# szemenyeim/DynEnv

Hardware: AMD Instinct MI355X
Metric: agent-steps/s (higher is better)
Workload: dtype f64

## Files before the change

### dynenv_amd/csrc/driving_kernels.hip

```cpp
#include "driving_dev.h"

__constant__ DrvConst C;

#include "driving_host.h"

struct DrvMailbox {
  double p1x[DRV_NS][2], p1y[DRV_NS][2], p2x[DRV_NS][2], p2y[DRV_NS][2], nx[DRV_NS], ny[DRV_NS];
  int hash[DRV_NS][2], count[DRV_NS], flag[DRV_NS];
};
struct DrvObsStage {
  float carRow[DRV_MAXA][8];
  float goal[DRV_MAXA][2];
  float shared[DRV_MAXO * 4 + DRV_MAXP * 2 + DRV_LANE_ROWS * 5];
};
#ifdef DRV_PROFILE
#define DRV_PROF(...) __VA_ARGS__
#else
#define DRV_PROF(...)
#endif
#define DRV_CLIST 128
struct __align__(16) DrvLds {
  double px[DRV_NB], py[DRV_NB], vx[DRV_NB], vy[DRV_NB], ang[DRV_NB], w[DRV_NB], vbx[DRV_NB], vby[DRV_NB], wb[DRV_NB];
  double minv[DRV_NB], iinv[DRV_NB];
  double rc[16], rs[16], rotAng[16];
  double dirx[16], diry[16], prevx[16], prevy[16], goalx[16], goaly[16];
  double cosRel0[16];
  double dprev[16];
  double cmass[16], cpower[16], chx[16], chy[16];
  double aabb[DRV_MAXA][4];
  int flags[DRV_NB], moving[DRV_NB];
  double ox[DRV_MAXO], oy[DRV_MAXO];
  int s_pair[DRV_NS], s_meta[DRV_NS], s_hash0[DRV_NS], s_hash1[DRV_NS];
  double s_jn0[DRV_NS], s_jt0[DRV_NS], s_jn1[DRV_NS], s_jt1[DRV_NS];
  double rewAcc[16], posAcc[16];
  int lastCand[64];
  int stepErr;
  unsigned char act[16];
  int still[DRV_NB];
  unsigned short clist[DRV_CLIST];
  int clistN;
  int sLvMeta;
  unsigned long long sActive;
  unsigned char sLevel[DRV_NS];
  union {
    DrvMailbox mb;
    DrvObsStage ob;
  } u;
};

static_assert(sizeof(DrvLds) <= 10240, "16 one-wave workgroups per CU - one residency round of 4096 environments on 256 CUs - need <= 160 KB / 16 of LDS each");
__shared__ DrvLds g_L;


#define DRV_COS_PI_2 6.123233995736766e-17
template <int R>
struct RoadK;
template <>
struct RoadK<0> {
  static constexpr double p0x = 875.0, p0y = 0.0, dirx = 0.0, diry = 1.0, lat = 2.0 * 35.0 + 5.0, length = 1000.0;
  static constexpr double dirAngle = 1.5707963267948966, cosDir0 = DRV_COS_PI_2, nx = -1.0, ny = DRV_COS_PI_2;
};
template <>
struct RoadK<1> {
  static constexpr double p0x = 0.0, p0y = 500.0, dirx = 1.0, diry = 0.0, lat = 1.0 * 35.0 + 5.0, length = 1750.0;
  static constexpr double dirAngle = 0.0, cosDir0 = 1.0, nx = DRV_COS_PI_2, ny = 1.0;
};

// ... 73 lines not shown
  const DevSC sc = INL ? dev_sincos_inl(ang) : dev_sincos(ang);
  CarRot r;
  r.c = sc.c; r.s = sc.s;
  r.cosRel0 = INL ? dev_sincos_inl(RoadK<0>::dirAngle - ang).c : dev_cos(RoadK<0>::dirAngle - ang);
  L.rc[lane] = r.c; L.rs[lane] = r.s; L.rotAng[lane] = ang; L.cosRel0[lane] = r.cosRel0;
  static_assert(RoadK<1>::dirAngle == 0.0, "cos(road1.dirAngle - angle) is read from rc");
  return r;
}

struct BoxW {
  V2 v[4], n[4];
};
DE_DEV void box_world(BoxW& b, V2 p, double rc, double rs, double hx, double hy) {
  const double lx[4] = {-hx, hx, hx, -hx}, ly[4] = {-hy, -hy, hy, hy};
  const double nx[4] = {-1.0, 0.0, 1.0, 0.0}, ny[4] = {0.0, -1.0, 0.0, 1.0};
#pragma unroll
  for (int i = 0; i < 4; ++i) {
    b.v[i] = v2(dms_xform_x(rc, rs, lx[i], ly[i], p.x), dms_xform_y(rc, rs, lx[i], ly[i], p.y));
    b.n[i] = v2(rc * nx[i] - rs * ny[i], rs * nx[i] + rc * ny[i]);
  }
}

struct Contacts {
  int count;
  V2 n, p1[2], p2[2];
  int hash[2];
};

struct EdgeW {
  V2 ap, bp, n;
  int ah, bh;
};

struct BoxP {
  V2 p;
  double c, s, hx, hy;
};
DE_DEV V2 boxp_vertex(const BoxP& b, int i) {
  const double lx = (i == 1 || i == 2) ? b.hx : -b.hx;
  const double ly = (i >= 2) ? b.hy : -b.hy;
  return v2(dms_xform_x(b.c, b.s, lx, ly, b.p.x), dms_xform_y(b.c, b.s, lx, ly, b.p.y));
}
DE_DEV V2 boxp_normal(const BoxP& b, int i) {
  const double nx = (i == 0) ? -1.0 : ((i == 2) ? 1.0 : 0.0);
  const double ny = (i == 1) ? -1.0 : ((i == 3) ? 1.0 : 0.0);
  return v2(b.c * nx - b.s * ny, b.s * nx + b.c * ny);
}

template <int S> DE_DEV double quad_bcast(double x) {
  int lo = __double2loint(x), hi = __double2hiint(x);
  lo = __builtin_amdgcn_update_dpp(lo, lo, S * 0x55, 0xF, 0xF, false);
  hi = __builtin_amdgcn_update_dpp(hi, hi, S * 0x55, 0xF, 0xF, false);
  return __hiloint2double(hi, lo);
}
DE_DEV void quad_argmax_first(double v, double& best, int& idx) {
  best = -INFINITY; idx = 0;
  double m;
  m = quad_bcast<0>(v); if (m > best) { best = m; idx = 0; }
  m = quad_bcast<1>(v); if (m > best) { best = m; idx = 1; }
  m = quad_bcast<2>(v); if (m > best) { best = m; idx = 2; }
  m = quad_bcast<3>(v); if (m > best) { best = m; idx = 3; }
}

DE_DEV int poly_support_index(const BoxP& p, V2 n, int q) {
  double mx;
  int index;
  quad_argmax_first(vdot_f(boxp_vertex(p, q), n), mx, index);
  return index;
}

DE_DEV EdgeW support_edge_poly(const BoxP& p, int slot, V2 n, int q) {
  int i1 = poly_support_index(p, n, q);
  int i0 = (i1 + 3) & 3;
  int i2 = (i1 + 1) & 3;
  int h = slot * 4;
  V2 n1 = boxp_normal(p, i1), n2 = boxp_normal(p, i2);
  EdgeW e;
  V2 vm = boxp_vertex(p, i1);
  if (vdot(n, n1) > vdot(n, n2)) {
    e.ap = boxp_vertex(p, i0); e.ah = h + i0; e.bp = vm; e.bh = h + i1; e.n = n1;
  } else {
    e.ap = vm; e.ah = h + i1; e.bp = boxp_vertex(p, i2); e.bh = h + i2; e.n = n2;
  }
  return e;
}

DE_DEV int hash_pair(int a, int b) { return 1 + ((a << 8) | b); }

DE_DEV void contact_points(const EdgeW& e1, const EdgeW& e2, V2 n, Contacts& out) {
  double d_e1_a = vcross(e1.ap, n), d_e1_b = vcross(e1.bp, n);
  double d_e2_a = vcross(e2.ap, n), d_e2_b = vcross(e2.bp, n);
  double e1_denom = 1.0 / (d_e1_b - d_e1_a + DE_DBL_MIN);
  double e2_denom = 1.0 / (d_e2_b - d_e2_a + DE_DBL_MIN);
  out.n = n;
  out.count = 0;
  {
    V2 p1 = vadd(vmul(n, 0.0), vlerp(e1.ap, e1.bp, fclamp01_cp((d_e2_b - d_e1_a) * e1_denom)));
    V2 p2 = vadd(vmul(n, -0.0), vlerp(e2.ap, e2.bp, fclamp01_cp((d_e1_a - d_e2_a) * e2_denom)));
    double dist = vdot(vsub(p2, p1), n);
    if (dist <= 0.0) { out.p1[0] = p1; out.p2[0] = p2; out.hash[0] = hash_pair(e1.ah, e2.bh); out.count = 1; }
  }
  {
    V2 p1 = vadd(vmul(n, 0.0), vlerp(e1.ap, e1.bp, fclamp01_cp((d_e2_a - d_e1_a) * e1_denom)));
    V2 p2 = vadd(vmul(n, -0.0), vlerp(e2.ap, e2.bp, fclamp01_cp((d_e1_b - d_e2_a) * e2_denom)));
    double dist = vdot(vsub(p2, p1), n);
    if (dist <= 0.0) {
      int h = hash_pair(e1.bh, e2.ah);
      if (out.count == 0) { out.p1[0] = p1; out.p2[0] = p2; out.hash[0] = h; }
      else { out.p1[1] = p1; out.p2[1] = p2; out.hash[1] = h; }
      out.count += 1;
    }
  }
}

DE_DEV double sat_max_sep(const BoxP& a, const BoxP& b, int q, int& best) {
  const V2 n = boxp_normal(a, q);
  const double d0 = vdot_f(n, boxp_vertex(a, q));
  double minv = INFINITY;
#pragma unroll
  for (int j = 0; j < 4; ++j) {
    double d = vdot_f(n, boxp_vertex(b, j)) - d0;
    if (d < minv) minv = d;
  }
  double maxsep;
  quad_argmax_first(minv, maxsep, best);
  return maxsep;
}

DE_DEV void poly_to_poly(const BoxP& p1, int slot1, const BoxP& p2, int slot2, int q, Contacts& out) {
  out.count = 0;
  int ia, ib;
  double sa = sat_max_sep(p1, p2, q, ia);
  if (sa > 0.0) return;
  double sb = sat_max_sep(p2, p1, q, ib);
  if (sb > 0.0) return;
  V2 n;
  if (sa >= sb) n = boxp_normal(p1, ia); else n = vneg(boxp_normal(p2, ib));
  const EdgeW e1 = support_edge_poly(p1, slot1, n, q);
  const EdgeW e2 = support_edge_poly(p2, slot2, vneg(n), q);
  contact_points(e1, e2, n, out);
}

DE_DEV void circle_to_poly(V2 c, double r, const BoxP& poly, int q, Contacts& out) {
  out.count = 0;
  double maxsep;
  int best;
  const V2 vq = boxp_vertex(poly, q);
  quad_argmax_first(vdot(boxp_normal(poly, q), vsub(c, vq)), maxsep, best);
  if (maxsep > r) return;
  if (maxsep <= 0.0) {
    V2 fn = boxp_normal(poly, best);
    V2 n = vneg(fn);
    V2 pb = vsub(c, vmul(fn, maxsep));
    out.n = n; out.p1[0] = vadd(c, vmul(n, r)); out.p2[0] = pb; out.hash[0] = 0; out.count = 1;
  } else {
    const V2 a = boxp_vertex(poly, (q + 3) & 3), b = vq;
    const V2 d = vsub(b, a);
    const double t = fclamp01_cp(vdot(d, vsub(c, a)) / vlensq(d));
    const V2 pt = vadd(a, vmul(d, t));
    const double dsq = vlensq(vsub(pt, c));
    double bestd = INFINITY;
    V2 bestp = c;
    double m;
    m = quad_bcast<0>(dsq); if (m < bestd) { bestd = m; bestp = v2(quad_bcast<0>(pt.x), quad_bcast<0>(pt.y)); }
    m = quad_bcast<1>(dsq); if (m < bestd) { bestd = m; bestp = v2(quad_bcast<1>(pt.x), quad_bcast<1>(pt.y)); }
    m = quad_bcast<2>(dsq); if (m < bestd) { bestd = m; bestp = v2(quad_bcast<2>(pt.x), quad_bcast<2>(pt.y)); }
    m = quad_bcast<3>(dsq); if (m < bestd) { bestd = m; bestp = v2(quad_bcast<3>(pt.x), quad_bcast<3>(pt.y)); }
    if (bestd <= r * r) {
      double dist = dm_sqrt(bestd);
      V2 delta = vsub(bestp, c);
      V2 n = (dist != 0.0) ? vmul(delta, 1.0 / dist) : vneg(boxp_normal(poly, best));
      out.n = n; out.p1[0] = vadd(c, vmul(n, r)); out.p2[0] = bestp; out.hash[0] = 0; out.count = 1;
    }
  }
}

struct BodyV {
  V2 p, v, vb;
  double w, wb, minv, iinv;
};
DE_DEV V2 static_pos(const DrvLds& L, int idx) {
  if (idx >= DRV_SLOT_BLD) {
    int k = idx - DRV_SLOT_BLD;
    return v2(DRV_BLD_CX(k), DRV_BLD_CY(k));
  }
  return v2(L.ox[idx - DRV_SLOT_OBST], L.oy[idx - DRV_SLOT_OBST]);
}
DE_DEV void body_load(const DrvLds& L, int idx, BodyV& b) {
  const bool dyn = idx < DRV_SLOT_OBST;
  const int bi = dyn ? idx : DRV_SLOT_OBST , oi = (idx >= DRV_SLOT_OBST && idx < DRV_SLOT_BLD) ? idx - DRV_SLOT_OBST : 0;
  const double dpx = L.px[bi], dpy = L.py[bi], sox = L.ox[oi], soy = L.oy[oi];
  const int k = idx - DRV_SLOT_BLD;
  const double bx = DRV_BLD_CX(k), by = DRV_BLD_CY(k);
  b.p = dyn ? v2(dpx, dpy) : (idx >= DRV_SLOT_BLD ? v2(bx, by) : v2(sox, soy));
  b.v = v2(L.vx[bi], L.vy[bi]); b.w = L.w[bi];
  b.vb = v2(L.vbx[bi], L.vby[bi]); b.wb = L.wb[bi]; b.minv = L.minv[bi]; b.iinv = L.iinv[bi];
}
DE_DEV void body_store_vel(DrvLds& L, int idx, const BodyV& b) {
  const int wi = idx < DRV_SLOT_OBST ? idx : DRV_NB - 1;
  L.vx[wi] = b.v.x; L.vy[wi] = b.v.y; L.w[wi] = b.w; L.vbx[wi] = b.vb.x; L.vby[wi] = b.vb.y; L.wb[wi] = b.wb;
}
DE_DEV double k_scalar_body(const BodyV& b, V2 r, V2 n) { return dms_k_scalar(b.minv, b.iinv, r.x, r.y, n.x, n.y); }
DE_DEV V2 relative_velocity(const BodyV& a, const BodyV& b, V2 r1, V2 r2) {
  V2 v1 = v2(dms_point_vx(a.v.x, r1.y, a.w), dms_point_vy(a.v.y, r1.x, a.w));
// ... 86 lines not shown
  const double g_px = b[BF_PX * E * DRV_NB], g_py = b[BF_PY * E * DRV_NB], g_vx = b[BF_VX * E * DRV_NB], g_vy = b[BF_VY * E * DRV_NB];
  const double g_ang = b[BF_ANG * E * DRV_NB], g_w = b[BF_W * E * DRV_NB];
  const double g_vbx = b[BF_VBX * E * DRV_NB], g_vby = b[BF_VBY * E * DRV_NB], g_wb = b[BF_WB * E * DRV_NB];
  const int g_f = S.flags[(size_t)e * DRV_NB + bl], g_aux = S.aux[(size_t)e * DRV_NB + bl];
  const double* c = S.carx + (size_t)e * 16 + cl;
  const double g_prevx = c[CF_PREVX * E * 16], g_prevy = c[CF_PREVY * E * 16], g_gx = c[CF_GOALX * E * 16], g_gy = c[CF_GOALY * E * 16];
  const double g_dirx = c[CF_DIRX * E * 16], g_diry = c[CF_DIRY * E * 16];
  const double g_ox = S.obst[(size_t)e * DRV_MAXO + ol], g_oy = S.obst[E * DRV_MAXO + (size_t)e * DRV_MAXO + ol];
  int g_pair = 0xFFFF, g_meta = 0, g_h0 = 0, g_h1 = 0;
  double g_jn0 = 0.0, g_jt0 = 0.0, g_jn1 = 0.0, g_jt1 = 0.0;
  if (occ != 0ull) {
    const size_t o = (size_t)e * DRV_NS + sl;
    g_pair = S.s_pair[o]; g_meta = S.s_meta[o];
    g_h0 = (int)S.s_hash[o]; g_h1 = (int)S.s_hash[E * DRV_NS + o];
    g_jn0 = S.s_imp[o]; g_jt0 = S.s_imp[E * DRV_NS + o]; g_jn1 = S.s_imp[2 * E * DRV_NS + o]; g_jt1 = S.s_imp[3 * E * DRV_NS + o];
  }
  if (lane < DRV_NB) {
    const bool used = lane < A || (lane >= DRV_SLOT_PED && lane < DRV_SLOT_PED + nPed);
    L.px[lane] = used ? g_px : 0.0; L.py[lane] = used ? g_py : 0.0;
    L.vx[lane] = used ? g_vx : 0.0; L.vy[lane] = used ? g_vy : 0.0;
    const double ang = used ? g_ang : 0.0;
    L.ang[lane] = ang; L.w[lane] = used ? g_w : 0.0;
    L.vbx[lane] = used ? g_vbx : 0.0; L.vby[lane] = used ? g_vby : 0.0;
    L.wb[lane] = used ? g_wb : 0.0;
    const int f = used ? g_f : 0;
    L.flags[lane] = f;
    L.moving[lane] = used ? g_aux : 0;
    const int ty = CARF_TYPE(f);
#define DRV_BY_TYPE(ARR) (ty == 3 ? CarK::ARR##3 : (ty == 2 ? CarK::ARR##2 : (ty == 1 ? CarK::ARR##1 : CarK::ARR##0)))
    double minv = 0.0, iinv = 0.0;
    if (lane < A) { minv = 1.0 / DRV_BY_TYPE(carMass); iinv = 1.0 / DRV_BY_TYPE(carInertia); }
    else if (used) { minv = 1.0 / CarK::pedMass; iinv = 1.0 / CarK::pedInertia; }
    L.minv[lane] = minv; L.iinv[lane] = iinv;
    if (lane < 16) { L.rc[lane] = 1.0; L.rs[lane] = 0.0; L.rotAng[lane] = 0.0; }
    if (lane < A) {
      L.dirx[lane] = g_dirx; L.diry[lane] = g_diry;
      L.prevx[lane] = g_prevx; L.prevy[lane] = g_prevy; L.goalx[lane] = g_gx; L.goaly[lane] = g_gy;
      L.dprev[lane] = vlen(vsub(v2(g_prevx, g_prevy), v2(g_gx, g_gy)));
      L.cmass[lane] = DRV_BY_TYPE(carMass); L.cpower[lane] = DRV_BY_TYPE(carPower);
      L.chx[lane] = DRV_BY_TYPE(carHx); L.chy[lane] = DRV_BY_TYPE(carHy);
      car_refresh_rot(L, lane, ang);
    }
#undef DRV_BY_TYPE
  }
  if (lane < DRV_MAXO) {
    L.ox[lane] = lane < nObst ? g_ox : 0.0;
    L.oy[lane] = lane < nObst ? g_oy : 0.0;
  }
  if (lane < DRV_NS) {
    const bool on = (occ >> lane) & 1ull;
    L.s_pair[lane] = on ? g_pair : 0xFFFF;
    L.s_meta[lane] = on ? g_meta : 0;
    L.s_hash0[lane] = on ? g_h0 : 0; L.s_hash1[lane] = on ? g_h1 : 0;
    L.s_jn0[lane] = on ? g_jn0 : 0.0; L.s_jt0[lane] = on ? g_jt0 : 0.0;
    L.s_jn1[lane] = on ? g_jn1 : 0.0; L.s_jt1[lane] = on ? g_jt1 : 0.0;
  }
}

DE_DEV void store_env(const DrvState& S, const DrvLds& L, int e, int lane, int A, int nPed, uint64_t occ) {
  const size_t E = (size_t)S.E;
  if (lane < A || (lane >= DRV_SLOT_PED && lane < DRV_SLOT_PED + nPed)) {
    double* b = S.body + (size_t)e * DRV_NB + lane;
    b[BF_PX * E * DRV_NB] = L.px[lane]; b[BF_PY * E * DRV_NB] = L.py[lane]; b[BF_VX * E * DRV_NB] = L.vx[lane];
    b[BF_VY * E * DRV_NB] = L.vy[lane]; b[BF_ANG * E * DRV_NB] = L.ang[lane]; b[BF_W * E * DRV_NB] = L.w[lane];
    b[BF_VBX * E * DRV_NB] = L.vbx[lane]; b[BF_VBY * E * DRV_NB] = L.vby[lane]; b[BF_WB * E * DRV_NB] = L.wb[lane];
    S.flags[(size_t)e * DRV_NB + lane] = L.flags[lane];
    if (lane < A) {
// ... 420 lines not shown
    const bool c = (bits >> i) & 1;
    const uint64_t m = wave_ballot(c);
    if (c) {
      const int idx = nCand + (int)__builtin_amdgcn_mbcnt_hi((uint32_t)(m >> 32), __builtin_amdgcn_mbcnt_lo((uint32_t)m, 0u));
      if (idx < DRV_CLIST) L.clist[idx] = (unsigned short)((i << 8) | lane); else err |= CRET_OVERFLOW;
    }
    nCand += __popcll(m);
  }
  savedN = mode == 1 && nCand <= DRV_CLIST ? nCand : -1;
  if (lane == 0) L.clistN = savedN;
  if (nCand > DRV_CLIST) nCand = DRV_CLIST;
  }
DRV_PROF(profCand += nCand;)
  __syncthreads();
DRV_PROF(const unsigned long long N1 = __builtin_amdgcn_s_memtime(); unsigned long long nMath = 0ull;)
  if (mode == 0) {
    bool owns = false;
    for (int k = lane; k < nCand; k += 64) {
      const int pr = (int)L.clist[k];
      for (uint64_t mm = occ; mm; mm &= mm - 1) owns = owns || bcast_i(spair, __builtin_ctzll(mm)) == pr;
    }
    if (wave_ballot(owns) != 0ull) continue;
  }
#pragma unroll 1
  for (int pass = 0; pass * 16 < nCand; ++pass) {
DRV_PROF(nMath -= __builtin_amdgcn_s_memtime();)
    const int q = lane & 3;
    const bool isCand = pass * 16 + (lane >> 2) < nCand;
    Contacts ct;
    ct.count = 0;
    const int pr = isCand ? (int)L.clist[pass * 16 + (lane >> 2)] : 0xFFFF;
    if (isCand) {
      const int i = pr >> 8, j = pr & 0xFF;
      BoxP b1;
      b1.p = v2(L.px[i], L.py[i]); b1.c = L.rc[i]; b1.s = L.rs[i]; b1.hx = L.chx[i]; b1.hy = L.chy[i];
      if (j >= DRV_SLOT_PED && j < DRV_SLOT_OBST) {
        circle_to_poly(v2(L.px[j], L.py[j]), DRV_PED_R, b1, q, ct);
      } else {
        BoxP b2;
        b2.c = 1.0; b2.s = 0.0;
        if (j < DRV_SLOT_PED) { b2.p = v2(L.px[j], L.py[j]); b2.c = L.rc[j]; b2.s = L.rs[j]; b2.hx = L.chx[j]; b2.hy = L.chy[j]; }
        else { b2.p = static_pos(L, j); b2.hx = j >= DRV_SLOT_BLD ? DRV_BLD_HX : DRV_OBST_H; b2.hy = j >= DRV_SLOT_BLD ? DRV_BLD_HY : DRV_OBST_H; }
        poly_to_poly(b1, i, b2, j, q, ct);
      }
    }
DRV_PROF(nMath += __builtin_amdgcn_s_memtime();)
    const bool touch = isCand && q == 0 && ct.count > 0;
    int slot = -1;
    if (mode != 0 && wave_ballot(touch) != 0ull) {
      for (uint64_t mm = occ; mm; mm &= mm - 1) {
        int sidx = __builtin_ctzll(mm);
        if (bcast_i(spair, sidx) == pr) slot = sidx;
      }
      if (!touch) slot = -1;
    }
    if (mode == 0) { lightBad = lightBad || touch; continue; }
    const uint64_t tmask = wave_ballot(touch);
    if (tmask == 0ull) continue;
    const bool needNew = touch && slot < 0;
    const uint64_t newMask = wave_ballot(needNew);
    if (newMask) {
      const uint64_t slotBits = (1ull << DRV_NS) - 1ull;
      int rank = __popcll(newMask & ((1ull << lane) - 1ull));
      uint64_t fm = (~occ) & slotBits;
      if (needNew) {
        for (int r = 0; r < rank; ++r) fm &= fm - 1;
        if (fm) { slot = __builtin_ctzll(fm); L.s_pair[slot] = pr; }
        else err |= CRET_OVERFLOW;
      }
      int cnt = __popcll(newMask);
      uint64_t fm2 = (~occ) & slotBits;
      for (int r = 0; r < cnt && fm2; ++r) { occ |= (fm2 & (~fm2 + 1)); fm2 &= fm2 - 1; }
      spair = lane < DRV_NS ? L.s_pair[lane] : -1;
    }
    if (touch && slot >= 0) {
// ... 215 lines not shown
  }
}

DE_OOL int drv_partial_obs_fused(PvIn in, uint64_t seed, int A, int* envi, int env_id_offset, int e, int nPedObst, int elapsed,
                                 uint32_t episode, int noiseTypeAgents, double magn, float* __restrict__ obs, int budgetCycles);
#ifndef DRV_DEFER_MIN_CONTACT
#define DRV_DEFER_MIN_CONTACT 5
#endif
#ifndef DRV_PV_DEADLINE_PCT
#define DRV_PV_DEADLINE_PCT 110
#endif
#ifndef DRV_FUSED_AGENTS
#define DRV_FUSED_AGENTS 10
#endif
enum { LR_MOVING = 1, LR_REMOVED = 2, LR_CAND_CHANGED = 4 };
enum { LS_VB_VALID = 1, LS_AABB_VALID = 2 };
struct DrvLightRet {
  int cand, dirty, bits;
};
DE_OOL DrvLightRet drv_light_substep(int it_, int lane, int A_, int nPed_, int nObst_, int elapsed_,
                                                      uint32_t seedLo, uint32_t seedHi, uint32_t genv_, uint32_t episode_, int stateBits) {
  DrvLds& L = g_L;
DRV_PROF(const unsigned long long Q0 = __builtin_amdgcn_s_memtime();)
  const int lastCand = L.lastCand[lane];
  const int it = uniform_i(it_), A = uniform_i(A_), nPed = uniform_i(nPed_), nObst = uniform_i(nObst_), elapsed = uniform_i(elapsed_);
  const uint32_t genv = (uint32_t)uniform_i((int)genv_), episode = (uint32_t)uniform_i((int)episode_);
  const uint64_t seed = ((uint64_t)(uint32_t)uniform_i((int)seedHi) << 32) | (uint64_t)(uint32_t)uniform_i((int)seedLo);
  const bool isCar = lane < A;
  const bool isPed = lane >= DRV_SLOT_PED && lane < DRV_SLOT_PED + nPed;
  const bool isBody = isCar || isPed;
  const bool vbValid = (uniform_i(stateBits) & LS_VB_VALID) != 0;
  bool aabbValid = (uniform_i(stateBits) & LS_AABB_VALID) != 0;
    bool turned = false;
    const int bi = lane & (DRV_NB - 1), ci = lane & 15;
    int f = L.flags[bi];
    double px = L.px[bi], py = L.py[bi], vx = L.vx[bi], vy = L.vy[bi], ang = L.ang[bi];
    const double w = L.w[bi];
    const double vbx = vbValid ? L.vbx[bi] : 0.0, vby = vbValid ? L.vby[bi] : 0.0, wb = vbValid ? L.wb[bi] : 0.0;
    double rcv = L.rc[ci], rsv = L.rs[ci], rotAngv = L.rotAng[ci], cosRel0v = L.cosRel0[ci];
    const double goalx = L.goalx[ci], goaly = L.goaly[ci], dprev = L.dprev[ci], chx = L.chx[ci], chy = L.chy[ci];
    double rew = L.rewAcc[ci], posrew = L.posAcc[ci];
    int moving = L.moving[bi];
    if (!isBody) { f = 0; px = 0.0; py = 0.0; vx = 0.0; vy = 0.0; }
    if (isCar) {
      if (it == 0) {
        const int actPk = (int)L.act[lane];
        const int acc = (actPk & 3) - 1, steer = ((actPk >> 2) - 1) * 2;
        if (!CARF_FIN(f)) {
          double dirx = L.dirx[lane], diry = L.diry[lane];
          double power = (double)acc;
          double moveDir = vx * dirx + vy * diry;
          bool skip = false;
          if (acc < 0) power = (double)acc * 0.75;
          if (acc == 0) power = (moveDir == 0.0) ? 0.0 : (moveDir > 0.0 ? -2.0 : 2.0);
          else if (acc < 0 && moveDir > 0.0) skip = true;
          else if (acc > 0 && moveDir < 0.0) skip = true;
          if (!skip) {
            const double cs = rcv, sn = rsv;
            const double cpower = L.cpower[lane];
            vx = vx + cpower * power * cs;
            vy = vy + cpower * power * sn;
            if (acc == 0 && (vx * dirx + vy * diry) * moveDir < 0.0) { vx = 0.0; vy = 0.0; }
          }
          if (steer != 0) {
            const double rot = (double)steer * (DM_PI / 180.0);
            ang = ang + rot;
            const DevSC rsc = dev_sincos_inl(rot);
// ... 83 lines not shown
          } else if (isOffRoad) {
            crossing = 0; beginc = 0;
          }
        }
        L.moving[lane] = moving;
        L.flags[lane] = PEDF_PACK(PEDF_ROAD(f), side, 0, crossing, beginc, PEDF_SPEED(f));
        L.vx[lane] = vx; L.vy[lane] = vy;
      }
    }

DRV_PROF(const unsigned long long Q3 = __builtin_amdgcn_s_memtime();)
    double bl = 0.0, bb = 0.0, br = -1.0, bt = -1.0;
    bool live = false;
    int sj = 3;
    if (isBody) {
      const double npx = px + (vx + vbx) * DE_DT, npy = py + (vy + vby) * DE_DT, nang = ang + (w + wb) * DE_DT;
      const bool still = !turned && vx == 0.0 && vy == 0.0 && w == 0.0 && vbx == 0.0 && vby == 0.0 && wb == 0.0;
      L.px[lane] = npx; L.py[lane] = npy; L.ang[lane] = nang;
      const bool frozen = !turned && vx == 0.0 && vy == 0.0 && w == 0.0 && npx == px && npy == py && nang == ang;
      sj = (still ? 1 : 0) | (frozen ? 2 : 0);
      L.still[lane] = sj;
      live = true;
      if (isCar) {
        if (nang != rotAngv) { const CarRot cr = car_refresh_rot<true>(L, lane, nang); rcv = cr.c; rsv = cr.s; }
        if (!aabbValid || !frozen) {
          BoxW bw;
          box_world(bw, v2(npx, npy), rcv, rsv, chx, chy);
          double l = INFINITY, r = -INFINITY, b = INFINITY, t = -INFINITY;
#pragma unroll
          for (int k = 0; k < 4; ++k) {
            l = fmin_cp(l, bw.v[k].x); r = fmax_cp(r, bw.v[k].x); b = fmin_cp(b, bw.v[k].y); t = fmax_cp(t, bw.v[k].y);
          }
          bl = l - 0.0; bb = b - 0.0; br = r + 0.0; bt = t + 0.0;
          L.aabb[lane][0] = bl; L.aabb[lane][1] = bb; L.aabb[lane][2] = br; L.aabb[lane][3] = bt;
        } else {
          bl = L.aabb[lane][0]; bb = L.aabb[lane][1]; br = L.aabb[lane][2]; bt = L.aabb[lane][3];
        }
      } else {
        bl = npx - DRV_PED_R; bb = npy - DRV_PED_R; br = npx + DRV_PED_R; bt = npy + DRV_PED_R;
      }
    } else if (lane >= DRV_SLOT_OBST && lane < DRV_SLOT_BLD + 4) {
      live = lane >= DRV_SLOT_BLD || (lane - DRV_SLOT_OBST) < nObst;
      const V2 c = static_pos(L, lane);
      const double ex = lane >= DRV_SLOT_BLD ? DRV_BLD_HX : DRV_OBST_H, ey = lane >= DRV_SLOT_BLD ? DRV_BLD_HY : DRV_OBST_H;
      bl = -ex + c.x; br = ex + c.x; bb = -ey + c.y; bt = ey + c.y;
    }
    aabbValid = true;
    __syncthreads();
DRV_PROF(const unsigned long long Q4 = __builtin_amdgcn_s_memtime();)

    int cand = 0;
    bool candMoving = false, removed = false;
    int dirty = 0;
    {
      const int carStill = (int)(wave_ballot(isCar && (sj & 1)) & 0x3FFull);
      const int carFrozen = (int)(wave_ballot(isCar && (sj & 2)) & 0x3FFull);
#pragma unroll
      for (int i = 0; i < DRV_MAXA; ++i) {
        const double al = L.aabb[i][0], ab = L.aabb[i][1], ar = L.aabb[i][2], at = L.aabb[i][3];
        const bool hit = (al <= br) & (bl <= ar) & (ab <= bt) & (bb <= at);
        cand |= hit ? (1 << i) : 0;
      }
      {
        const int lim = lane < A ? lane : A;
        cand &= live ? ((1 << lim) - 1) : 0;
      }
// ... 123 lines not shown
  if (mask && uniform_i(mask[e]) == 0) {
    if ((S.iso_on == 1 || S.iso_on == 2) && lane == 0) __atomic_store_n(&S.iso_done[e], tick, __ATOMIC_RELAXED);
    return;
  }
DRV_PROF(if (lane < 8 && e < 4096) { g_dbgp[e * 8 + lane] = 0ull; g_dbgs[e * 8 + lane] = 0ull; })
  const int A = S.A;
  int* envi = S.envi + (size_t)e * EI_COUNT;
  int elapsed = uniform_i(envi[EI_ELAPSED]);
  int allFinished = uniform_i(envi[EI_ALLFIN]);
  const int nPed = uniform_i(envi[EI_NPED]);
  const int nObst = uniform_i(envi[EI_NOBST]);
  const uint32_t episode = (uint32_t)uniform_i(envi[EI_EPISODE]);
  uint64_t occ = (uint64_t)(uint32_t)uniform_i(envi[EI_OCC]);
  if (occ != 0ull) __builtin_amdgcn_s_setprio(3);
  else if (PARTIAL) __builtin_amdgcn_s_setprio(1);
  const uint32_t genv = (uint32_t)(S.env_id_offset + e);

  const bool isCar = lane < A;
  const bool isPed = lane >= DRV_SLOT_PED && lane < DRV_SLOT_PED + nPed;
  const bool isBody = isCar || isPed;
  const int g_act0 = actions[((size_t)e * A + (isCar ? lane : 0)) * 2 + 0], g_act1 = actions[((size_t)e * A + (isCar ? lane : 0)) * 2 + 1];
  const int g_lastCand = S.lastcand[(size_t)e * 64 + lane];
  load_env(S, L, e, lane, A, nPed, nObst, occ);

  {
    int act0 = isCar ? g_act0 : 1, act1 = isCar ? g_act1 : 1;
    const bool bad = (unsigned)act0 > 2u || (unsigned)act1 > 2u;
    if (bad) { act0 = 1; act1 = 1; }
    if (lane < 16) L.act[lane] = (unsigned char)(act0 | (act1 << 2));
    const bool anyBad = wave_ballot(bad) != 0ull;
    if (lane == 0) L.stepErr = anyBad ? DYNENV_ERRBIT_ACTION : 0;
  }
  int finishedAt = -1;
  if (lane < 16) { L.rewAcc[lane] = 0.0; L.posAcc[lane] = 0.0; }
  bool aabbValid = false;
  L.lastCand[lane] = g_lastCand;
  if (lane == 0) { L.clistN = -1; L.sActive = ~0ull; L.sLvMeta = 0; }
  bool inertAll = (uniform_i(envi[EI_SHORTCUT]) & SC_INERT) != 0;
  bool steadyAll = (uniform_i(envi[EI_SHORTCUT]) & SC_STEADY) != 0;
  bool vbValid = (uniform_i(envi[EI_SHORTCUT]) & SC_VB_VALID) != 0;
  unsigned cntA = 0u, cntB = 0u;
#define DRV_CNT(ei) (1u << (4 * ((ei) - EI_N_FAST)))
#define DRV_CNT_GET(ei) ((int)((cntA >> (4 * ((ei) - EI_N_FAST))) & 15u))
  static_assert(EI_N_STEADY - EI_N_FAST == 7 && EI_N_SLOTS - EI_N_FAST == 3 && DRV_NS * 10 < 256, "seven counters of four bits in cntA, the slot sum in eight bits of cntB");
  __syncthreads();

DRV_PROF(const unsigned long long K0 = __builtin_amdgcn_s_memtime(); unsigned long long tPh1 = 0, tBroad = 0, tFast = 0, tCont = 0, tBook = 0;)
  bool lightOff = false;
  for (int it = 0; it < 10; ++it) {
    lane = fresh_lane();
DRV_PROF(const unsigned long long A0 = __builtin_amdgcn_s_memtime();)
    const DrvLightRet lr = drv_light_substep(it, lane, A, nPed, nObst, elapsed, (uint32_t)S.seed, (uint32_t)(S.seed >> 32), genv, episode,
                                             (vbValid ? LS_VB_VALID : 0) | (aabbValid ? LS_AABB_VALID : 0));
    const int cand = lr.cand, dirty = lr.dirty;
    const bool candMoving = (lr.bits & LR_MOVING) != 0, removed = (lr.bits & LR_REMOVED) != 0;
    aabbValid = true;
DRV_PROF(const unsigned long long A1 = A0;)
    const uint64_t anyCand = wave_ballot(cand != 0);
    const bool candChanged = wave_ballot((lr.bits & LR_CAND_CHANGED) != 0) != 0ull, anyMoving = wave_ballot(candMoving) != 0ull;
    if (candChanged && lane == 0) L.clistN = -1;
    const bool quiescent = inertAll && !candChanged && !anyMoving;
    const bool steadyOk = !quiescent && steadyAll && wave_ballot(removed) == 0ull;
    const bool anyDirty = wave_ballot(dirty != 0) != 0ull;
    bool replay = steadyOk && !anyDirty;
    const bool light = steadyOk && anyDirty && !lightOff;
    if (!(anyCand == 0ull && occ == 0ull) && !quiescent && !replay) cntA += candChanged ? DRV_CNT(EI_N_WHY_CAND) : anyMoving ? DRV_CNT(EI_N_WHY_MOVING) : DRV_CNT(EI_N_WHY_INERT);

// ... 285 lines not shown
```

Measured before the change: 270.3 million.

## Cache car world-space corners in LDS and split contact clipping across quad lanes

After: 273.1 million (median of 6 runs). 1.0% higher.

```diff
diff --git a/dynenv_amd/csrc/driving_kernels.hip b/dynenv_amd/csrc/driving_kernels.hip
--- a/dynenv_amd/csrc/driving_kernels.hip
+++ b/dynenv_amd/csrc/driving_kernels.hip
@@ -22,17 +22,18 @@
 struct __align__(16) DrvLds {
   double px[DRV_NB], py[DRV_NB], vx[DRV_NB], vy[DRV_NB], ang[DRV_NB], w[DRV_NB], vbx[DRV_NB], vby[DRV_NB], wb[DRV_NB];
   double minv[DRV_NB], iinv[DRV_NB];
-  double rc[16], rs[16], rotAng[16];
-  double dirx[16], diry[16], prevx[16], prevy[16], goalx[16], goaly[16];
-  double cosRel0[16];
-  double dprev[16];
-  double cmass[16], cpower[16], chx[16], chy[16];
+  double rc[DRV_MAXA], rs[DRV_MAXA], rotAng[DRV_MAXA];
+  double dirx[DRV_MAXA], diry[DRV_MAXA], prevx[DRV_MAXA], prevy[DRV_MAXA], goalx[DRV_MAXA], goaly[DRV_MAXA];
+  double cosRel0[DRV_MAXA];
+  double dprev[DRV_MAXA];
+  double cmass[DRV_MAXA], cpower[DRV_MAXA], chx[DRV_MAXA], chy[DRV_MAXA];
   double aabb[DRV_MAXA][4];
+  V2 cv[DRV_MAXA][4];
   int flags[DRV_NB], moving[DRV_NB];
   double ox[DRV_MAXO], oy[DRV_MAXO];
   int s_pair[DRV_NS], s_meta[DRV_NS], s_hash0[DRV_NS], s_hash1[DRV_NS];
   double s_jn0[DRV_NS], s_jt0[DRV_NS], s_jn1[DRV_NS], s_jt1[DRV_NS];
-  double rewAcc[16], posAcc[16];
+  double rewAcc[DRV_MAXA], posAcc[DRV_MAXA];
   int lastCand[64];
   int stepErr;
   unsigned char act[16];
@@ -172,16 +173,27 @@
   int ah, bh;
 };
 
-struct BoxP {
-  V2 p;
-  double c, s, hx, hy;
+struct BoxC {
+  V2 v[4], vq;
+  double c, s;
 };
-DE_DEV V2 boxp_vertex(const BoxP& b, int i) {
-  const double lx = (i == 1 || i == 2) ? b.hx : -b.hx;
-  const double ly = (i >= 2) ? b.hy : -b.hy;
-  return v2(dms_xform_x(b.c, b.s, lx, ly, b.p.x), dms_xform_y(b.c, b.s, lx, ly, b.p.y));
-}
-DE_DEV V2 boxp_normal(const BoxP& b, int i) {
+DE_DEV void boxc_car(const DrvLds& L, int i, int q, BoxC& b) {
+#pragma unroll
+  for (int k = 0; k < 4; ++k) b.v[k] = L.cv[i][k];
+  b.vq = L.cv[i][q];
+  b.c = L.rc[i]; b.s = L.rs[i];
+}
+DE_DEV void boxc_static(V2 p, double hx, double hy, int q, BoxC& b) {
+  const double x0 = -hx + p.x, x1 = hx + p.x, y0 = -hy + p.y, y1 = hy + p.y;
+  b.v[0] = v2(x0, y0); b.v[1] = v2(x1, y0); b.v[2] = v2(x1, y1); b.v[3] = v2(x0, y1);
+  b.vq = v2((q == 1 || q == 2) ? x1 : x0, (q >= 2) ? y1 : y0);
+  b.c = 1.0; b.s = 0.0;
+}
+DE_DEV V2 boxc_vertex(const BoxC& b, int i) {
+  const V2 v0 = b.v[0], v1 = b.v[1], v2_ = b.v[2], v3 = b.v[3];
+  return v2(i == 0 ? v0.x : (i == 1 ? v1.x : (i == 2 ? v2_.x : v3.x)), i == 0 ? v0.y : (i == 1 ? v1.y : (i == 2 ? v2_.y : v3.y)));
+}
+DE_DEV V2 boxc_normal(const BoxC& b, int i) {
   const double nx = (i == 0) ? -1.0 : ((i == 2) ? 1.0 : 0.0);
   const double ny = (i == 1) ? -1.0 : ((i == 3) ? 1.0 : 0.0);
   return v2(b.c * nx - b.s * ny, b.s * nx + b.c * ny);
@@ -193,6 +205,7 @@
   hi = __builtin_amdgcn_update_dpp(hi, hi, S * 0x55, 0xF, 0xF, false);
   return __hiloint2double(hi, lo);
 }
+template <int S> DE_DEV int quad_bcast_i(int x) { return __builtin_amdgcn_update_dpp(x, x, S * 0x55, 0xF, 0xF, false); }
 DE_DEV void quad_argmax_first(double v, double& best, int& idx) {
   best = -INFINITY; idx = 0;
   double m;
@@ -202,64 +215,53 @@
   m = quad_bcast<3>(v); if (m > best) { best = m; idx = 3; }
 }
 
-DE_DEV int poly_support_index(const BoxP& p, V2 n, int q) {
+DE_DEV int poly_support_index(const BoxC& p, V2 n) {
   double mx;
   int index;
-  quad_argmax_first(vdot_f(boxp_vertex(p, q), n), mx, index);
+  quad_argmax_first(vdot_f(p.vq, n), mx, index);
   return index;
 }
 
-DE_DEV EdgeW support_edge_poly(const BoxP& p, int slot, V2 n, int q) {
-  int i1 = poly_support_index(p, n, q);
-  int i0 = (i1 + 3) & 3;
-  int i2 = (i1 + 1) & 3;
-  int h = slot * 4;
-  V2 n1 = boxp_normal(p, i1), n2 = boxp_normal(p, i2);
+DE_DEV EdgeW support_edge_poly(const BoxC& p, int slot, V2 n) {
+  const int i1 = poly_support_index(p, n);
+  const int i2 = (i1 + 1) & 3;
+  const int h = slot * 4;
+  const V2 n1 = boxc_normal(p, i1), n2 = boxc_normal(p, i2);
+  const bool front = vdot(n, n1) > vdot(n, n2);
+  const int ib = front ? i1 : i2, ia = (ib + 3) & 3;
   EdgeW e;
-  V2 vm = boxp_vertex(p, i1);
-  if (vdot(n, n1) > vdot(n, n2)) {
-    e.ap = boxp_vertex(p, i0); e.ah = h + i0; e.bp = vm; e.bh = h + i1; e.n = n1;
-  } else {
-    e.ap = vm; e.ah = h + i1; e.bp = boxp_vertex(p, i2); e.bh = h + i2; e.n = n2;
-  }
+  e.ap = boxc_vertex(p, ia); e.ah = h + ia; e.bp = boxc_vertex(p, ib); e.bh = h + ib; e.n = v2(front ? n1.x : n2.x, front ? n1.y : n2.y);
   return e;
 }
 
 DE_DEV int hash_pair(int a, int b) { return 1 + ((a << 8) | b); }
 
-DE_DEV void contact_points(const EdgeW& e1, const EdgeW& e2, V2 n, Contacts& out) {
-  double d_e1_a = vcross(e1.ap, n), d_e1_b = vcross(e1.bp, n);
-  double d_e2_a = vcross(e2.ap, n), d_e2_b = vcross(e2.bp, n);
-  double e1_denom = 1.0 / (d_e1_b - d_e1_a + DE_DBL_MIN);
-  double e2_denom = 1.0 / (d_e2_b - d_e2_a + DE_DBL_MIN);
+DE_DEV void contact_points(const EdgeW& e1, const EdgeW& e2, V2 n, int q, Contacts& out) {
+  const bool odd = (q & 1) != 0;
+  const double d_e1_a = vcross(e1.ap, n), d_e1_b = vcross(e1.bp, n);
+  const double d_e2_a = vcross(e2.ap, n), d_e2_b = vcross(e2.bp, n);
+  const double denom = 1.0 / ((odd ? d_e2_b : d_e1_b) - (odd ? d_e2_a : d_e1_a) + DE_DBL_MIN);
+  const double e1_denom = quad_bcast<0>(denom), e2_denom = quad_bcast<1>(denom);
+  const V2 p1 = vadd(vmul(n, 0.0), vlerp(e1.ap, e1.bp, fclamp01_cp(((odd ? d_e2_a : d_e2_b) - d_e1_a) * e1_denom)));
+  const V2 p2 = vadd(vmul(n, -0.0), vlerp(e2.ap, e2.bp, fclamp01_cp(((odd ? d_e1_b : d_e1_a) - d_e2_a) * e2_denom)));
+  const int hit = vdot(vsub(p2, p1), n) <= 0.0 ? 1 : 0;
+  const bool hitA = quad_bcast_i<0>(hit) != 0, hitB = quad_bcast_i<1>(hit) != 0;
+  const V2 p1B = v2(quad_bcast<1>(p1.x), quad_bcast<1>(p1.y)), p2B = v2(quad_bcast<1>(p2.x), quad_bcast<1>(p2.y));
+  const int hA = hash_pair(e1.ah, e2.bh), hB = hash_pair(e1.bh, e2.ah);
   out.n = n;
-  out.count = 0;
-  {
-    V2 p1 = vadd(vmul(n, 0.0), vlerp(e1.ap, e1.bp, fclamp01_cp((d_e2_b - d_e1_a) * e1_denom)));
-    V2 p2 = vadd(vmul(n, -0.0), vlerp(e2.ap, e2.bp, fclamp01_cp((d_e1_a - d_e2_a) * e2_denom)));
-    double dist = vdot(vsub(p2, p1), n);
-    if (dist <= 0.0) { out.p1[0] = p1; out.p2[0] = p2; out.hash[0] = hash_pair(e1.ah, e2.bh); out.count = 1; }
-  }
-  {
-    V2 p1 = vadd(vmul(n, 0.0), vlerp(e1.ap, e1.bp, fclamp01_cp((d_e2_a - d_e1_a) * e1_denom)));
-    V2 p2 = vadd(vmul(n, -0.0), vlerp(e2.ap, e2.bp, fclamp01_cp((d_e1_b - d_e2_a) * e2_denom)));
-    double dist = vdot(vsub(p2, p1), n);
-    if (dist <= 0.0) {
-      int h = hash_pair(e1.bh, e2.ah);
-      if (out.count == 0) { out.p1[0] = p1; out.p2[0] = p2; out.hash[0] = h; }
-      else { out.p1[1] = p1; out.p2[1] = p2; out.hash[1] = h; }
-      out.count += 1;
-    }
-  }
-}
-
-DE_DEV double sat_max_sep(const BoxP& a, const BoxP& b, int q, int& best) {
-  const V2 n = boxp_normal(a, q);
-  const double d0 = vdot_f(n, boxp_vertex(a, q));
+  out.count = (hitA ? 1 : 0) + (hitB ? 1 : 0);
+  out.p1[0] = v2(hitA ? p1.x : p1B.x, hitA ? p1.y : p1B.y); out.p2[0] = v2(hitA ? p2.x : p2B.x, hitA ? p2.y : p2B.y);
+  out.hash[0] = hitA ? hA : hB;
+  out.p1[1] = p1B; out.p2[1] = p2B; out.hash[1] = hB;
+}
+
+DE_DEV double sat_max_sep(const BoxC& a, const BoxC& b, int q, int& best) {
+  const V2 n = boxc_normal(a, q);
+  const double d0 = vdot_f(n, a.vq);
   double minv = INFINITY;
 #pragma unroll
   for (int j = 0; j < 4; ++j) {
-    double d = vdot_f(n, boxp_vertex(b, j)) - d0;
+    double d = vdot_f(n, b.v[j]) - d0;
     if (d < minv) minv = d;
   }
   double maxsep;
@@ -267,7 +269,7 @@
   return maxsep;
 }
 
-DE_DEV void poly_to_poly(const BoxP& p1, int slot1, const BoxP& p2, int slot2, int q, Contacts& out) {
+DE_DEV void poly_to_poly(const BoxC& p1, int slot1, const BoxC& p2, int slot2, int q, Contacts& out) {
   out.count = 0;
   int ia, ib;
   double sa = sat_max_sep(p1, p2, q, ia);
@@ -275,26 +277,26 @@
   double sb = sat_max_sep(p2, p1, q, ib);
   if (sb > 0.0) return;
   V2 n;
-  if (sa >= sb) n = boxp_normal(p1, ia); else n = vneg(boxp_normal(p2, ib));
-  const EdgeW e1 = support_edge_poly(p1, slot1, n, q);
-  const EdgeW e2 = support_edge_poly(p2, slot2, vneg(n), q);
-  contact_points(e1, e2, n, out);
-}
-
-DE_DEV void circle_to_poly(V2 c, double r, const BoxP& poly, int q, Contacts& out) {
+  if (sa >= sb) n = boxc_normal(p1, ia); else n = vneg(boxc_normal(p2, ib));
+  const EdgeW e1 = support_edge_poly(p1, slot1, n);
+  const EdgeW e2 = support_edge_poly(p2, slot2, vneg(n));
+  contact_points(e1, e2, n, q, out);
+}
+
+DE_DEV void circle_to_poly(V2 c, double r, const BoxC& poly, V2 vp, int q, Contacts& out) {
   out.count = 0;
   double maxsep;
   int best;
-  const V2 vq = boxp_vertex(poly, q);
-  quad_argmax_first(vdot(boxp_normal(poly, q), vsub(c, vq)), maxsep, best);
+  const V2 vq = poly.vq;
+  quad_argmax_first(vdot(boxc_normal(poly, q), vsub(c, vq)), maxsep, best);
   if (maxsep > r) return;
   if (maxsep <= 0.0) {
-    V2 fn = boxp_normal(poly, best);
+    V2 fn = boxc_normal(poly, best);
     V2 n = vneg(fn);
     V2 pb = vsub(c, vmul(fn, maxsep));
     out.n = n; out.p1[0] = vadd(c, vmul(n, r)); out.p2[0] = pb; out.hash[0] = 0; out.count = 1;
   } else {
-    const V2 a = boxp_vertex(poly, (q + 3) & 3), b = vq;
+    const V2 a = vp, b = vq;
     const V2 d = vsub(b, a);
     const double t = fclamp01_cp(vdot(d, vsub(c, a)) / vlensq(d));
     const V2 pt = vadd(a, vmul(d, t));
@@ -309,7 +311,7 @@
     if (bestd <= r * r) {
       double dist = dm_sqrt(bestd);
       V2 delta = vsub(bestp, c);
-      V2 n = (dist != 0.0) ? vmul(delta, 1.0 / dist) : vneg(boxp_normal(poly, best));
+      V2 n = (dist != 0.0) ? vmul(delta, 1.0 / dist) : vneg(boxc_normal(poly, best));
       out.n = n; out.p1[0] = vadd(c, vmul(n, r)); out.p2[0] = bestp; out.hash[0] = 0; out.count = 1;
     }
   }
@@ -462,7 +464,7 @@
     if (lane < A) { minv = 1.0 / DRV_BY_TYPE(carMass); iinv = 1.0 / DRV_BY_TYPE(carInertia); }
     else if (used) { minv = 1.0 / CarK::pedMass; iinv = 1.0 / CarK::pedInertia; }
     L.minv[lane] = minv; L.iinv[lane] = iinv;
-    if (lane < 16) { L.rc[lane] = 1.0; L.rs[lane] = 0.0; L.rotAng[lane] = 0.0; }
+    if (lane < DRV_MAXA) { L.rc[lane] = 1.0; L.rs[lane] = 0.0; L.rotAng[lane] = 0.0; }
     if (lane < A) {
       L.dirx[lane] = g_dirx; L.diry[lane] = g_diry;
       L.prevx[lane] = g_prevx; L.prevy[lane] = g_prevy; L.goalx[lane] = g_gx; L.goaly[lane] = g_gy;
@@ -949,15 +951,14 @@
     const int pr = isCand ? (int)L.clist[pass * 16 + (lane >> 2)] : 0xFFFF;
     if (isCand) {
       const int i = pr >> 8, j = pr & 0xFF;
-      BoxP b1;
-      b1.p = v2(L.px[i], L.py[i]); b1.c = L.rc[i]; b1.s = L.rs[i]; b1.hx = L.chx[i]; b1.hy = L.chy[i];
+      BoxC b1;
+      boxc_car(L, i, q, b1);
       if (j >= DRV_SLOT_PED && j < DRV_SLOT_OBST) {
-        circle_to_poly(v2(L.px[j], L.py[j]), DRV_PED_R, b1, q, ct);
+        circle_to_poly(v2(L.px[j], L.py[j]), DRV_PED_R, b1, L.cv[i][(q + 3) & 3], q, ct);
       } else {
-        BoxP b2;
-        b2.c = 1.0; b2.s = 0.0;
-        if (j < DRV_SLOT_PED) { b2.p = v2(L.px[j], L.py[j]); b2.c = L.rc[j]; b2.s = L.rs[j]; b2.hx = L.chx[j]; b2.hy = L.chy[j]; }
-        else { b2.p = static_pos(L, j); b2.hx = j >= DRV_SLOT_BLD ? DRV_BLD_HX : DRV_OBST_H; b2.hy = j >= DRV_SLOT_BLD ? DRV_BLD_HY : DRV_OBST_H; }
+        BoxC b2;
+        if (j < DRV_SLOT_PED) boxc_car(L, j, q, b2);
+        else boxc_static(static_pos(L, j), j >= DRV_SLOT_BLD ? DRV_BLD_HX : DRV_OBST_H, j >= DRV_SLOT_BLD ? DRV_BLD_HY : DRV_OBST_H, q, b2);
         poly_to_poly(b1, i, b2, j, q, ct);
       }
     }
@@ -1239,7 +1240,7 @@
   const bool vbValid = (uniform_i(stateBits) & LS_VB_VALID) != 0;
   bool aabbValid = (uniform_i(stateBits) & LS_AABB_VALID) != 0;
     bool turned = false;
-    const int bi = lane & (DRV_NB - 1), ci = lane & 15;
+    const int bi = lane & (DRV_NB - 1), ci = lane < DRV_MAXA ? lane : DRV_MAXA - 1;
     int f = L.flags[bi];
     double px = L.px[bi], py = L.py[bi], vx = L.vx[bi], vy = L.vy[bi], ang = L.ang[bi];
     const double w = L.w[bi];
@@ -1389,6 +1390,8 @@
             l = fmin_cp(l, bw.v[k].x); r = fmax_cp(r, bw.v[k].x); b = fmin_cp(b, bw.v[k].y); t = fmax_cp(t, bw.v[k].y);
           }
           bl = l - 0.0; bb = b - 0.0; br = r + 0.0; bt = t + 0.0;
+#pragma unroll
+          for (int k = 0; k < 4; ++k) L.cv[lane][k] = bw.v[k];
           L.aabb[lane][0] = bl; L.aabb[lane][1] = bb; L.aabb[lane][2] = br; L.aabb[lane][3] = bt;
         } else {
           bl = L.aabb[lane][0]; bb = L.aabb[lane][1]; br = L.aabb[lane][2]; bt = L.aabb[lane][3];
@@ -1578,7 +1581,7 @@
     if (lane == 0) L.stepErr = anyBad ? DYNENV_ERRBIT_ACTION : 0;
   }
   int finishedAt = -1;
-  if (lane < 16) { L.rewAcc[lane] = 0.0; L.posAcc[lane] = 0.0; }
+  if (lane < DRV_MAXA) { L.rewAcc[lane] = 0.0; L.posAcc[lane] = 0.0; }
   bool aabbValid = false;
   L.lastCand[lane] = g_lastCand;
   if (lane == 0) { L.clistN = -1; L.sActive = ~0ull; L.sLvMeta = 0; }
```
